# nubomedia/NUBOMEDIA-VCA

Measured on AMD Instinct MI355X. Metric: 1080p frames/sec/node (NuboFaceDetector); achieved HBM GB/s vs peak, higher is better.
Workload: dtype i32 rect sums / f32 products / f64 stage sums (u8 pixels)

## Files before the change

### nubomedia-vca_amd/csrc/device_records.h

```cpp
#pragma once
#include <stdint.h>
#include <stddef.h>

#if defined(__HIPCC__)
#define NVCA_HD __host__ __device__
#else
#define NVCA_HD
#endif

namespace nvca {

struct StageRec {
    int first, count; float thr;
    int flags;
    int thr_i;
    int vote_exp;
    int spec_run;
    int pad1;
};

struct ScaleRec {
    int    winw, winh;
    int    plane_off;
    int    pitch;
    int    endX, endY;
    int    eq[4];
    int    xpos_off, ypos_off;
    int    sq32;
    int    task_off;
    int    wpr;
    int    adaptive;
    double inv_area;
    double factor;
    const struct TStumpRec *trecs;
    const struct GNodeRec *grecs;
    const struct LStumpRec *lrecs;
};

struct GNodeRec {
    short dx[3][4], dy[3][4];
    float w[3];
    float thr;
    int left, right;
    int flags;
    int pad;
};
static_assert(sizeof(GNodeRec) == 80, "GNodeRec layout");

struct StripRec { int scale, iy0, nrows, ix0, ncols, pad0, pad1, pad2; };
struct TileRec {
    int scale, ix0, iy0, nx, ny;
    int x0, y0;
    int ncol, nrow;
    int span_x, span_y;
    int col_off, row_off;
    int pad_t;
    int pad0, pad1;
};
struct TStumpRec {
    int x0[3], x1[3], y0[3], y1[3];
    float w[3];
    int nrect;
    double thr, a0, a1;
    int a0i, a1i;
};
static_assert(sizeof(TStumpRec) == 96, "TStumpRec layout is read dword by dword in kernels_cascade_tile.hip");
struct alignas(16) LStumpRec {
    unsigned xx0, yy0, xx1, yy1, xx2, yy2;
    float w0, w1, w2, thr, a0, a1;
};
static_assert(sizeof(LStumpRec) == 48, "LStumpRec is read as three int4 in kernels_cascade_tile.hip");
struct DeepRec { int col_off, ncol, row_off, nrow, span_x, span_y, pad0, pad1; };
static constexpr int kDeepMaxSide = 64;
static constexpr int kDeepMaxSpan = 1280;
struct BandRec { int scale, iy0, ny, first_tile, ntiles, pad0, pad1, pad2; };
static constexpr int kTileWin = 32;
static constexpr int kTileRows = 16;
static constexpr int kTileSlots = kTileWin * kTileRows;
static constexpr int kTileThreads = kTileSlots;
static constexpr int kTilesPerCu = 3;
static constexpr int kTileWavesPerSimd = (kTilesPerCu * kTileThreads / 64 + 3) / 4;
static constexpr int kTileLdsBudget = 52 * 1024;
static_assert(kTilesPerCu * kTileLdsBudget <= 160 * 1024 && kTilesPerCu * kTileThreads <= 32 * 64, "tile residency per CU");
static constexpr int kTileMaxCols = 256;
NVCA_HD inline int tile_pitch(int ncol) { return ncol | 1; }
NVCA_HD inline int tile_lds_fixed()
{
    return kTileSlots * 8 + 2 * kTileSlots * 2 + 4 * kTileWin + 128 + kTileSlots * 8;
}
NVCA_HD inline int tile_lds_bytes(int ncol, int nrow, int span_x, int span_y)
{
    return 4 * nrow * tile_pitch(ncol) + 2 * ((span_x + 3) & ~3) + 2 * ((span_y + 3) & ~3) + tile_lds_fixed();
}

static constexpr int kStripMaxWin = 512;
static constexpr int kIntegralBand = 16;

struct PreGeom {
    int sw, sh, sstride, cn;
    int w, h, gpitch;
    int spitch;
    int nbands;
    size_t src_slot, gray_slot, sum_slot, band_slot;
};
struct YuvPlanes {
    int fmt, cstride, vstride, pad;
    long long off_y, off_u, off_v;
};
struct ResizeView {
    int mode, xmax;
    const int *xofs; const short *ialpha; const int *yofs; const short *ibeta;
};
struct PyrLevelDev {
    int szw, szh, gpitch, plane_off;
    long long gray_off;
    ResizeView tab;
};

struct TrkSlot {
    const uint8_t *src;
    uint8_t *prev;
    float *mhi;
    float ts, delbound;
    float seg;
    int threshold;
    int has_prev;
    int sstride;
    int min_area;
    long long max_area;
    YuvPlanes yuv;
};
struct CompAcc { int minx, miny, maxx, maxy, seed, pad; };
inline size_t tracker_count_offset(int w, int h, int batch) { return ((size_t)((w + 255) / 256) * h * batch + 63) & ~(size_t)63; }
inline size_t tracker_flag_bytes(int w, int h, int batch) { return tracker_count_offset(w, h, batch) + sizeof(int) * (size_t)batch; }

struct CascadeArgs {
    const int *sum; const unsigned long long *sqsum;
    size_t sum_slot;
    int spitch;
    const ScaleRec *scales; const StageRec *stages;
    const StripRec *strips; const int *pos;
    const int *order; int blocks_per_frame;
    const TileRec *tiles; const int *tile_order; int tile_blocks_per_frame;
    const unsigned short *tcoords; int tile_lds;
    const BandRec *bands; const int *band_order; int band_blocks_per_frame; int batch; int band_map;
    const DeepRec *deeprecs;
    int nscales;
    const unsigned *tasks; int ntasks;
    unsigned long long *failbits;
    double *vnf;
    int nstages; int pair_policy;
    int stage_order;
    int *stage_hint;
    int spec_pairs;
    int pair_max;
    const float *stage_thr;
    const int *stage_first;
    int deep_stage;
    int deep_lds;
    unsigned long long *deep;
    unsigned deep_cap;
    int key_sy, key_ss;
    unsigned long long *hits;
    unsigned hit_cap;
    const int *tilted;
    const float *galpha;
    const int *gcls_first;
    int stump_based;
#ifdef NVCA_STAMPS
    unsigned long long *dbg;
#endif
};

struct LbpWeakDev { int off[16]; int subset[8]; float leaf[2]; int pad[6]; };
static_assert(sizeof(LbpWeakDev) == 128, "LbpWeakDev is fetched with wide scalar loads");
struct LbpStageDev { int first, count; float thr; int pad; };
struct LbpLevelDev { int plane_off, szw, szh, nx, ny, step, wpr, bit_off, row_first, pad0, pad1, pad2; };
struct LbpTile { int level, tx, ty, pad; };
static constexpr int kLbpTileW = 32, kLbpTileH = 16;
NVCA_HD inline int lbp_tile_pitch(int ow) { return (kLbpTileW - 1) * 2 + ow + 1; }
NVCA_HD inline int lbp_tile_rows(int oh, int step) { return (kLbpTileH - 1) * step + oh + 1; }
struct LbpArgs {
    const int *sum;
    int P, TP;
    int ow, oh;
    const LbpLevelDev *levels; int nlev;
    const LbpStageDev *stages; int nstages;
    const LbpWeakDev *gweak, *tweak;
    const LbpTile *tiles; int ntiles;
    unsigned *bits, *bits2;
    int tile_stages;
    int nrows;
    int key_sy, key_ss;
    unsigned *cnt;
    unsigned *list[2]; unsigned list_cap;
    unsigned long long *hits; unsigned hit_cap;
};

struct RoiStep {
    const TStumpRec *trecs;
    int ex, ey, ew, eh;
    int startX, endX, startY, endY;
    int step, adaptive, job, key_step;
    int key_x0, key_dx, key_y0, key_dy;
    int szw, szh;
    int mode, xmax, xofs_off, yofs_off, ialpha_off, ibeta_off;
    double inv_area, ystep;
    int rej_off, rej_wpr;
};
struct RoiJobDev {
    const uint8_t *img; int w, h, stride;
    int first_step, nsteps, scale_image;
    const StageRec *stages; int nstages, pair_policy;
    int slot, pad;
};
static constexpr int kRoiMaxWin = 2048;

}
```

### nubomedia-vca_amd/csrc/kernels_cascade_tile.hip

```cpp
#include "launch.h"
#include "cascade_device.h"
#include <mutex>

namespace nvca {

template <class T> __device__ __forceinline__ T load_const(const T *p)
{
    static_assert(sizeof(T) % 4 == 0, "dword records only");
    typedef const __attribute__((address_space(4))) int CInt;
    CInt *q = (CInt *)p;
    T r;
    int *d = (int *)&r;
#pragma unroll
    for (int i = 0; i < (int)(sizeof(T) / 4); i++) d[i] = q[i];
    return r;
}

struct ScaleHot {
    int plane_off, pitch, eq[4], xpos_off, ypos_off, sq32, task_off, wpr, adaptive;
    double inv_area;
    const TStumpRec *trecs; const LStumpRec *lrecs;
};
__device__ __forceinline__ ScaleHot load_scale(const ScaleRec *p)
{
    typedef const __attribute__((address_space(4))) ScaleRec CScaleRec;
    CScaleRec *q = (CScaleRec *)p;
    ScaleHot h;
    h.plane_off = q->plane_off; h.pitch = q->pitch;
#pragma unroll
    for (int i = 0; i < 4; i++) h.eq[i] = q->eq[i];
    h.xpos_off = q->xpos_off; h.ypos_off = q->ypos_off; h.sq32 = q->sq32; h.task_off = q->task_off; h.wpr = q->wpr; h.adaptive = q->adaptive;
    h.inv_area = q->inv_area;
    h.trecs = q->trecs; h.lrecs = q->lrecs;
    return h;
}
struct TileScale {
    int pitch, xpos_off, ypos_off, wpr;
    const char *sum;
    double *vnf;
    const TStumpRec *trecs; const LStumpRec *lrecs;
};
__device__ __forceinline__ TileScale tile_scale(const CascadeArgs &a, const ScaleHot &h, int slot)
{
    TileScale ts;
    ts.pitch = h.pitch; ts.xpos_off = h.xpos_off; ts.ypos_off = h.ypos_off; ts.wpr = h.wpr;
    ts.sum = (const char *)(a.sum + (size_t)slot * a.sum_slot + h.plane_off);
    ts.vnf = a.vnf + ((size_t)slot * a.ntasks + h.task_off) * 64;
    ts.trecs = h.trecs; ts.lrecs = h.lrecs;
    return ts;
}


typedef int int16v __attribute__((ext_vector_type(16)));
typedef int int8v __attribute__((ext_vector_type(8)));
struct SRec { int16v a; int8v b; };
__device__ __forceinline__ SRec load_srec(const TStumpRec *p)
{
    SRec r;
    asm volatile("s_load_dwordx16 %0, %2, 0x0\n\ts_load_dwordx8 %1, %2, 0x40\n\ts_waitcnt lgkmcnt(0)"
                 : "=&s"(r.a), "=&s"(r.b) : "s"(p) : "memory");
    return r;
}
typedef __attribute__((address_space(1))) const void *gptr_t;
typedef __attribute__((address_space(3))) void *lptr_t;
typedef __attribute__((address_space(3))) const unsigned short lds_cu16;
typedef __attribute__((address_space(3))) const int lds_ci32;
#pragma clang diagnostic push
#pragma clang diagnostic ignored "-Wint-to-pointer-cast"
__device__ __forceinline__ unsigned lds_addr(const void *p) { return (unsigned)(unsigned long long)(lptr_t)p; }
__device__ __forceinline__ int lds_u16(unsigned a) { return *(lds_cu16 *)a; }
__device__ __forceinline__ int lds_sample(int r, int c)
{
    unsigned a;
    asm("v_lshl_add_u32 %0, %1, 2, %2" : "=v"(a) : "v"(r), "v"(c));
    return *(lds_ci32 *)a;
}
#pragma clang diagnostic pop
template <bool PAIR, class Sum>
__device__ __forceinline__ Sum tile_vote_s(unsigned cm, unsigned rm, double vnf, const SRec &f)
{
    const int share = f.a[15] >> 8;
    const int ca = lds_u16(cm + 2 * f.a[0]), cb = lds_u16(cm + 2 * f.a[3]);
    const int ra = lds_u16(rm + 2 * f.a[6]), rb = lds_u16(rm + 2 * f.a[9]);
    auto rs = [&](int x0, int x1, int y0, int y1, int sh) {
        int c0 = ca, c1 = cb, r0 = ra, r1 = rb;
        if (!(sh & 2)) { c0 = lds_u16(cm + 2 * x0); c1 = lds_u16(cm + 2 * x1); }
        if (!(sh & 1)) { r0 = lds_u16(rm + 2 * y0); r1 = lds_u16(rm + 2 * y1); }
        return lds_sample(r0, c0) - lds_sample(r0, c1) - lds_sample(r1, c0) + lds_sample(r1, c1);
    };
    const int s0 = lds_sample(ra, ca) - lds_sample(ra, cb) - lds_sample(rb, ca) + lds_sample(rb, cb);
    const int s1 = rs(f.a[1], f.a[4], f.a[7], f.a[10], share);
    const double t = __hiloint2double(f.b[1], f.b[0]) * vnf;
    const float w0 = __int_as_float(f.a[12]), w1 = __int_as_float(f.a[13]);
    double v;
    if (PAIR) {
        const float fs = (float)s0 * w0 + (float)s1 * w1;
        v = (double)fs;
    } else {
        v = (double)((float)s0 * w0);
        v += (double)((float)s1 * w1);
        if ((f.a[15] & 255) == 3) {
            const int s2 = rs(f.a[2], f.a[5], f.a[8], f.a[11], share >> 2);
            v += (double)((float)s2 * __int_as_float(f.a[14]));
        }
    }
    if (sizeof(Sum) == sizeof(int)) return (Sum)(v >= t ? f.b[7] : f.b[6]);
    const double a0 = __hiloint2double(f.b[3], f.b[2]), a1 = __hiloint2double(f.b[5], f.b[4]);
    return (Sum)(v >= t ? a1 : a0);
}
template <bool PAIR, class Sum = double>
__device__ __forceinline__ Sum tile_stage_sum(unsigned cm, unsigned rm, double vnf, const TStumpRec *recs, int j0, int count, int step)
{
    const TStumpRec *base = recs;
    asm("" : "+v"(cm), "+v"(rm));
    Sum sum = 0;
    for (int j = j0; j < count; j += step) sum += tile_vote_s<PAIR, Sum>(cm, rm, vnf, load_srec(base + j));
    return sum;
}
__device__ __forceinline__ bool tile_stage_pass(unsigned cm, unsigned rm, double vnf, const TStumpRec *recs, const StageRec &st, bool pair)
{
    if (st.flags & 4) {
        const int sum = pair ? tile_stage_sum<true, int>(cm, rm, vnf, recs + st.first, 0, st.count, 1) : tile_stage_sum<false, int>(cm, rm, vnf, recs + st.first, 0, st.count, 1);
        return sum >= st.thr_i;
    }
    const double sum = pair ? tile_stage_sum<true>(cm, rm, vnf, recs + st.first, 0, st.count, 1) : tile_stage_sum<false>(cm, rm, vnf, recs + st.first, 0, st.count, 1);
    return !(sum < (double)st.thr);
}

struct LRec { int4 a, b, c; };
__device__ __forceinline__ LRec load_lrec(const LStumpRec *p)
{
    const int4 *q = (const int4 *)p;
    LRec r; r.a = q[0]; r.b = q[1]; r.c = q[2];
    return r;
}
__device__ __forceinline__ int lane_rect(unsigned cm, unsigned rm, unsigned xx, unsigned yy)
{
    const int c0 = lds_u16(cm + (xx & 0xffffu)), c1 = lds_u16(cm + (xx >> 16));
    const int r0 = lds_u16(rm + (yy & 0xffffu)), r1 = lds_u16(rm + (yy >> 16));
    return lds_sample(r0, c0) - lds_sample(r0, c1) - lds_sample(r1, c0) + lds_sample(r1, c1);
}
__device__ __forceinline__ double lane_vote(unsigned cm, unsigned rm, double vnf, const LRec &f, int pair_policy)
{
    const int s0 = lane_rect(cm, rm, (unsigned)f.a.x, (unsigned)f.a.y);
    const int s1 = lane_rect(cm, rm, (unsigned)f.a.z, (unsigned)f.a.w);
    const double t = (double)__int_as_float(f.c.y) * vnf;
    const float p0 = (float)s0 * __int_as_float(f.b.z), p1 = (float)s1 * __int_as_float(f.b.w);
    double v = (double)p0;
    v += (double)p1;
    if (f.b.x) v += (double)((float)lane_rect(cm, rm, (unsigned)f.b.x, (unsigned)f.b.y) * __int_as_float(f.c.x));
    else if (pair_policy && f.b.y == 1) v = (double)(p0 + p1);
    return (double)__int_as_float(v >= t ? f.c.w : f.c.z);
}

#ifdef NVCA_STAMPS
#define NVCA_STAMP(a, tile, id) do { if (threadIdx.x == 0 && blockIdx.x < 64 && (tile) < 16 && (id) < 64 && (a).dbg) { unsigned long long t__; \
    asm volatile("s_memtime %0\n\ts_waitcnt lgkmcnt(0)" : "=s"(t__) :: "memory"); (a).dbg[((size_t)blockIdx.x * 16 + (tile)) * 64 + (id)] = t__; } } while (0)
#define NVCA_STAMP_VAL(a, tile, id, v) do { if (threadIdx.x == 0 && blockIdx.x < 64 && (tile) < 16 && (id) < 64 && (a).dbg) (a).dbg[((size_t)blockIdx.x * 16 + (tile)) * 64 + (id)] = (unsigned long long)(v); } while (0)
#else
#define NVCA_STAMP(a, tile, id) do { } while (0)
#define NVCA_STAMP_VAL(a, tile, id, v) do { } while (0)
#endif

struct TileLds {
    double *acc;
    unsigned short *q0, *winx, *winy; int *qn; double *vnf_s;
    unsigned short *cmap, *rmap; int *T; int pitchT;
    int tword;
    unsigned cmA, rmA;
};
__device__ __forceinline__ TileLds carve_tile(unsigned char *lds, const TileRec &t)
{
    TileLds L;
    L.acc = (double *)lds;
    L.q0 = (unsigned short *)(lds + kTileSlots * 8);
    L.winx = L.q0 + 2 * kTileSlots; L.winy = L.winx + kTileWin;
    L.qn = (int *)(L.winy + kTileWin);
    L.vnf_s = (double *)((unsigned char *)L.qn + 128);
    L.cmap = (unsigned short *)(L.vnf_s + kTileSlots);
    L.rmap = L.cmap + ((t.span_x + 3) & ~3);
    L.T = (int *)(L.rmap + ((t.span_y + 3) & ~3));
    L.pitchT = tile_pitch(t.ncol);
    L.tword = (int)(lds_addr(L.T) >> 2);
    L.cmA = lds_addr(L.cmap); L.rmA = lds_addr(L.rmap);
    return L;
}

struct TileCoords { int mapc, mapr, wx, wy; unsigned rowy, xc[4]; };
__device__ __forceinline__ TileCoords tile_coords(const CascadeArgs &a, const TileRec &t, const TileScale &sc)
{
    const int tid = threadIdx.x, lane = tid & 63, wave = tid >> 6;
    constexpr int NW = kTileThreads / 64;
    const unsigned short *__restrict__ cl = a.tcoords + t.col_off, *__restrict__ rl = a.tcoords + t.row_off;
    TileCoords c;
    c.mapc = tid < t.ncol ? (int)cl[tid] : -1;
    c.mapr = tid < t.nrow ? (int)rl[tid] : -1;
    c.wx = tid < t.nx ? a.pos[sc.xpos_off + t.ix0 + tid] : 0;
    c.wy = (tid >= 64 && tid < 64 + t.ny) ? a.pos[sc.ypos_off + t.iy0 + tid - 64] : 0;
    const int nmine = t.nrow > wave ? (t.nrow - wave + NW - 1) / NW : 0;
    c.rowy = 0u;
    if (lane < nmine) c.rowy = rl[wave + NW * lane];
#pragma unroll
    for (int k = 0; k < 4; k++) { const int q = lane + 64 * k; c.xc[k] = cl[q < t.ncol ? q : t.ncol - 1]; }
    return c;
}
__device__ __forceinline__ void tile_commit(const TileRec &t, const TileScale &sc, const TileLds &L, const TileCoords &c)
{
    const int tid = threadIdx.x, lane = tid & 63, wave = __builtin_amdgcn_readfirstlane(tid >> 6);
    constexpr int NW = kTileThreads / 64;
    const char *__restrict__ src = sc.sum;
    const int nmine = t.nrow > wave ? (t.nrow - wave + NW - 1) / NW : 0;
    const int nk = (t.ncol + 63) >> 6;
    for (int j = 0; j < nmine; j++) {
        const unsigned rb = (unsigned)__builtin_amdgcn_readlane((int)c.rowy, j) * (unsigned)sc.pitch * 4u;
        const char *rowp = src + rb;
        int *dst = L.T + (wave + NW * j) * L.pitchT;
#pragma unroll
        for (int k = 0; k < 4; k++)
            if (k < nk && lane + 64 * k < t.ncol)
                __builtin_amdgcn_global_load_lds((gptr_t)(rowp + 4u * c.xc[k]), (lptr_t)(dst + 64 * k), 4, 0, 0);
    }
    if (tid < 3) L.qn[tid] = 0;
    if (tid < t.nx) L.winx[tid] = (unsigned short)(c.wx - t.x0);
    if (tid >= 64 && tid < 64 + t.ny) L.winy[tid - 64] = (unsigned short)(c.wy - t.y0);
    if (c.mapc >= 0) L.cmap[c.mapc - t.x0] = (unsigned short)(tid * 4);
    if (c.mapr >= 0) L.rmap[c.mapr - t.y0] = (unsigned short)(L.tword + tid * L.pitchT);
}

__device__ __forceinline__ void queue_push_wave0(bool keep, int w, unsigned short *q, int *count)
{
    if (threadIdx.x >= 64) return;
    const int lane = threadIdx.x;
    const unsigned long long km = __ballot(keep);
    if (keep) q[__popcll(km & ((1ull << lane) - 1ull))] = (unsigned short)w;
    if (lane == 0) *count = __popcll(km);
}
__device__ __forceinline__ void queue_push(bool keep, int w, unsigned short *q, int *count)
{
    const int lane = threadIdx.x & 63;
    const unsigned long long km = __ballot(keep);
    if (km) {
        int wbase = 0;
        if (lane == 0) wbase = atomicAdd(count, __popcll(km));
        wbase = __shfl(wbase, 0);
        if (keep) q[wbase + __popcll(km & ((1ull << lane) - 1ull))] = (unsigned short)w;
    }
}

static constexpr int kStatStages = 6;
static constexpr int kPairMax = 32;
static_assert(7 * kPairMax <= kTileSlots && 64 + kTileRows <= kTileThreads && kTileRows <= kTileWin,
              "a round's seven accumulator rows fit the tile's accumulators; threads 64 .. 64 + kTileRows - 1 fill winy[kTileWin]");
template <bool VNF_LDS>
__device__ __forceinline__ void tile_stages(const CascadeArgs &a, const TileRec &t, const TileScale &sc, int slot, const TileLds &L, int ti = 0, int par = 0)
{
    const int tid = threadIdx.x, lane = tid & 63;
    const int wave = __builtin_amdgcn_readfirstlane(tid >> 6);
    const int *stat_r = L.qn + 4 + par * kStatStages;
    int *stat_w = L.qn + 4 + (par ^ 1) * kStatStages;
    constexpr int NW = kTileThreads / 64;
    const TStumpRec *urecs = sc.trecs;
    const double *__restrict__ vnfp = sc.vnf + (size_t)t.iy0 * sc.wpr * 64;
    auto vnf_of = [&](int w) {
        if (VNF_LDS) return L.vnf_s[w];
        const int ix = t.ix0 + (w & 31);
        return vnfp[((size_t)(w >> 5) * sc.wpr + (ix >> 6)) * 64 + (ix & 63)];
    };
    int *acci = (int *)L.acc;
    int cur = 0;
    int cin = 0;
    const int last = a.deep_stage < a.nstages ? a.deep_stage : a.nstages;
    const int m = (last < kStatStages ? last : kStatStages) - 1;
    const bool adapt = a.stage_order && m >= 2;
    unsigned ordpack = 0x54321u;
    if (adapt) {
        const unsigned o = (unsigned)__builtin_amdgcn_readfirstlane(stat_r[0]);
        unsigned seen = 0;
        for (int q = 0; q < m; q++) seen |= 1u << ((o >> (4 * q)) & 15u);
        if (seen == (2u << m) - 2u) ordpack = o;
    }
    int kpos = 0, prev = 0; unsigned entered = 0;
    auto stage_at = [&](int kp) { return __builtin_amdgcn_readfirstlane((adapt && kp < m) ? (int)((ordpack >> (4 * kp)) & 15u) : kp + 1); };
    struct I8 { int v[8]; };
    struct F8 { float v[8]; };
    const int s_first = last > 1 ? stage_at(0) : 0;
    StageRec st = load_const(a.stages + s_first);
    I8 F = load_const((const I8 *)(a.stage_first + s_first));
    F8 TH = load_const((const F8 *)(a.stage_thr + s_first));
    while (kpos < last - 1) {
        const bool in_prefix = adapt && kpos < m;
        const int s = stage_at(kpos);
        __syncthreads();
        NVCA_STAMP(a, ti, 8 + 8 * s);
        const int n = __builtin_amdgcn_readfirstlane(L.qn[cin]);
        if (adapt && tid == 0 && prev) stat_w[prev] |= n;
        if (n == 0) break;
        NVCA_STAMP_VAL(a, ti, 8 + 8 * s + 7, n);
        const int cout = cin == 2 ? 0 : cin + 1;
        if (tid == 0) L.qn[cout == 2 ? 0 : cout + 1] = 0;
        const unsigned short *qi = L.q0 + cur * kTileSlots;
        unsigned short *qo = L.q0 + (cur ^ 1) * kTileSlots;
        const bool pair = a.pair_policy && (st.flags & 1);
        int adv = 1;
        if (n <= a.pair_max && (st.flags & 2)) {
            const int G = 64 / n;
            int mm = 1;
            if (!in_prefix) {
                int lim = st.spec_run < last - s ? st.spec_run : last - s;
                if (lim > 7) lim = 7;
#pragma unroll
                for (int q = 1; q < 7; q++)
                    if (mm == q && q < lim && n * (F.v[q + 1] - F.v[0]) <= a.spec_pairs) mm = q + 1;
            }
            const int g0 = F.v[0];
            int g1 = F.v[1];
#pragma unroll
            for (int q = 2; q < 8; q++) if (mm >= q) g1 = F.v[q];
            const unsigned inv = 65535u / (unsigned)n + 1u;
            const int cc = (int)(((unsigned)lane * inv) >> 16), j = lane - cc * n;
            if (cc < G) {
                const int w = qi[j];
                const unsigned cm = L.cmA + 2 * L.winx[w & 31], rm = L.rmA + 2 * L.winy[w >> 5];
                const double vnf = vnf_of(w);
                for (int g = g0 + wave * G + cc; g < g1; g += NW * G) {
                    const LRec f = load_lrec(sc.lrecs + g);
                    const int r = (g >= F.v[1]) + (g >= F.v[2]) + (g >= F.v[3]) + (g >= F.v[4]) + (g >= F.v[5]) + (g >= F.v[6]);
                    atomicAdd(&L.acc[r * kPairMax + j], lane_vote(cm, rm, vnf, f, a.pair_policy));
                }
            }
            NVCA_STAMP(a, ti, 8 + 8 * s + 1);
            __syncthreads();
            NVCA_STAMP(a, ti, 8 + 8 * s + 2);
            bool pass = false; int w = 0;
            if (tid < n) {
                pass = true;
#pragma unroll
                for (int r = 0; r < 7; r++)
                    if (r < mm) {
                        const double sum = L.acc[r * kPairMax + tid];
                        L.acc[r * kPairMax + tid] = 0.;
                        pass = pass && !(sum < (double)TH.v[r]);
                    }
                w = qi[tid];
            }
            if (s < kStatStages && tid == 0) stat_w[s] = adapt ? n << 16 : n;
            queue_push_wave0(pass, w, qo, &L.qn[cout]);
            adv = mm;
            NVCA_STAMP(a, ti, 8 + 8 * s + 3);
        } else if (st.flags & 6) {
            const bool ints = (st.flags & 4) != 0;
            const int C = st.count;
            const int rem = n & 63, nfull = n >> 6;
            const bool rem_pair = rem > 0 && rem <= a.pair_max;
            const int Gr = rem_pair ? 64 / rem : 1;
            const int lead = (rem_pair ? nfull : (n + 63) >> 6) * C;
            const int items = lead + (rem_pair ? (C + Gr - 1) / Gr : 0), K = (items + NW - 1) / NW;
            const double vscale = ints ? __hiloint2double((1023 - st.vote_exp) << 20, 0) : 1.;
            int e = wave * K;
            const int e1 = e + K < items ? e + K : items;
            while (e < e1 && e < lead) {
                const int top = e1 < lead ? e1 : lead;
                const int wg = e / C, c0 = e - wg * C, c1 = (C - c0 < top - e) ? C : c0 + (top - e);
                const int i = wg * 64 + lane;
                if (i < n) {
                    const int w = qi[i];
                    const int xw = L.winx[w & 31], yw = L.winy[w >> 5];
                    const double vnf = vnf_of(w);
                    const unsigned cm = L.cmA + 2 * xw, rm = L.rmA + 2 * yw;
                    if (ints) {
                        const int v = pair ? tile_stage_sum<true, int>(cm, rm, vnf, urecs + st.first, c0, c1, 1) : tile_stage_sum<false, int>(cm, rm, vnf, urecs + st.first, c0, c1, 1);
                        atomicAdd(&acci[i], v);
                    } else {
                        const double v = pair ? tile_stage_sum<true, double>(cm, rm, vnf, urecs + st.first, c0, c1, 1) : tile_stage_sum<false, double>(cm, rm, vnf, urecs + st.first, c0, c1, 1);
                        atomicAdd(&L.acc[i], v);
                    }
                }
                e += c1 - c0;
            }
            if (e < e1) {
                const unsigned inv = 65535u / (unsigned)rem + 1u;
                const int cc = (int)(((unsigned)lane * inv) >> 16), j = lane - cc * rem;
                if (cc < Gr) {
                    const int i = nfull * 64 + j;
                    const int w = qi[i];
                    const unsigned cm = L.cmA + 2 * L.winx[w & 31], rm = L.rmA + 2 * L.winy[w >> 5];
                    const double vnf = vnf_of(w);
                    double sum = 0.;
                    for (int c = (e - lead) * Gr + cc; c < (e1 - lead) * Gr && c < C; c += Gr)
                        sum += lane_vote(cm, rm, vnf, load_lrec(sc.lrecs + st.first + c), a.pair_policy);
                    if (ints) atomicAdd(&acci[i], (int)(sum * vscale)); else atomicAdd(&L.acc[i], sum);
                }
            }
            NVCA_STAMP(a, ti, 8 + 8 * s + 1);
            __syncthreads();
            NVCA_STAMP(a, ti, 8 + 8 * s + 2);
            bool pass = false; int w = 0;
            if (tid < n) {
                if (ints) { const int sa = acci[tid]; acci[tid] = 0; pass = sa >= st.thr_i; }
                else { const double sa = L.acc[tid]; L.acc[tid] = 0.; pass = !(sa < (double)st.thr); }
                w = qi[tid];
            }
            if (s < kStatStages && tid == 0) stat_w[s] = adapt ? n << 16 : n;
            if (n <= 64) queue_push_wave0(pass, w, qo, &L.qn[cout]); else queue_push(pass, w, qo, &L.qn[cout]);
            NVCA_STAMP(a, ti, 8 + 8 * s + 3);
        } else {
            for (int base = 0; base < n; base += kTileThreads) {
                const int i = base + tid;
                bool pass = false; int w = 0;
                if (i < n) {
                    w = qi[i];
                    const int xw = L.winx[w & 31], yw = L.winy[w >> 5];
                    const double vnf = vnf_of(w);
                    pass = tile_stage_pass(L.cmA + 2 * xw, L.rmA + 2 * yw, vnf, urecs, st, pair);
                }
                queue_push(pass, w, qo, &L.qn[cout]);
            }
            if (tid == 0 && s < kStatStages) stat_w[s] = adapt ? n << 16 : n;
        }
        cur ^= 1; cin = cout;
        if (in_prefix) { prev = s; entered |= 1u << s; } else prev = 0;
        kpos += adv;
        if (kpos < last - 1) {
            const int sn = stage_at(kpos);
            st = load_const(a.stages + sn); F = load_const((const I8 *)(a.stage_first + sn)); TH = load_const((const F8 *)(a.stage_thr + sn));
        }
    }
    __syncthreads();
    NVCA_STAMP(a, ti, 6);
    const int nh = L.qn[cin];
    if (adapt && tid == 0) {
        if (prev) stat_w[prev] |= nh;
        int key[kStatStages - 1], id[kStatStages - 1];
        bool known = true;
#pragma unroll
        for (int q = 1; q < kStatStages; q++) {
            int v = stat_w[q];
            const int old = stat_r[q];
            if (q <= m && (!((entered >> q) & 1u) || ((v >> 16) < 16 && old != 0))) { v = old; stat_w[q] = v; }
            const int ent = v >> 16, pas = v & 0xffff, cnt = L.qn[4 + 2 * kStatStages - 1 + q] ;
            if (q <= m && ent == 0) known = false;
            const int killed = ent - pas > 0 ? ent - pas : 0;
            key[q - 1] = q > m ? 0x7fffffff : (killed ? (cnt * ent * 64) / killed : 0x7ffffff0);
            id[q - 1] = q;
        }
#pragma unroll
        for (int pass_i = 0; pass_i < kStatStages - 2; pass_i++)
#pragma unroll
            for (int q = 0; q + 1 < kStatStages - 1 - pass_i; q++)
                if (key[q] / 2 > key[q + 1]) { const int tk = key[q];        key[q] = key[q + 1]; key[q + 1] = tk; const int ti2 = id[q]; id[q] = id[q + 1]; id[q + 1] = ti2; }
        unsigned pack = 0;
#pragma unroll
        for (int q = 0; q < kStatStages - 1; q++) pack |= (unsigned)id[q] << (4 * q);
        stat_w[0] = known ? (int)pack : 0;
        if (known && a.stage_hint) {
#pragma unroll
            for (int q = 1; q < kStatStages; q++) a.stage_hint[q] = stat_w[q];
            a.stage_hint[0] = (int)pack;
        }
    }
    if (nh == 0) return;
    unsigned long long *list = last == a.nstages ? a.hits : a.deep;
    const unsigned cap = last == a.nstages ? a.hit_cap : a.deep_cap;
    if (tid == 0) L.qn[3] = (int)(unsigned)atomicAdd(list, (unsigned long long)nh);
    __syncthreads();
    const unsigned gb = (unsigned)L.qn[3];
    const unsigned short *qi = L.q0 + cur * kTileSlots;
    for (int i = tid; i < nh; i += kTileThreads) {
        const int w = qi[i], ix = t.ix0 + (w & 31);
        const unsigned key = ((unsigned)t.scale << a.key_ss) | ((unsigned)(t.iy0 + (w >> 5)) << a.key_sy) | (unsigned)ix;
        if (gb + i < cap) list[1 + gb + i] = ((unsigned long long)slot << 32) | key;
        if (VNF_LDS && last != a.nstages) sc.vnf[((size_t)(t.iy0 + (w >> 5)) * sc.wpr + (ix >> 6)) * 64 + (ix & 63)] = L.vnf_s[w];
    }
    NVCA_STAMP(a, ti, 7);
}

__device__ __forceinline__ void tile_prologue(const CascadeArgs &a, const TileLds &L)
{
    const int tid = threadIdx.x;
    L.acc[tid] = 0.;
    if (tid < 2 * kStatStages) L.qn[4 + tid] = (tid < kStatStages && a.stage_hint) ? a.stage_hint[tid] : 0;
    if (tid >= 1 && tid < kStatStages) L.qn[4 + 2 * kStatStages - 1 + tid] = tid < a.nstages ? a.stages[tid].count : 0;
}

__global__ __launch_bounds__(kTileThreads, kTileWavesPerSimd) void k_tile(CascadeArgs a)
{
    extern __shared__ __align__(16) unsigned char lds[];
    const int tid = threadIdx.x;
    const int slot = blockIdx.x / a.tile_blocks_per_frame;
    const int tidx = a.tile_order[blockIdx.x - slot * a.tile_blocks_per_frame];
    if (tidx < 0) return;
    const TileRec t = a.tiles[tidx];
    const ScaleHot sh = load_scale(a.scales + t.scale);
    const TileScale sc = tile_scale(a, sh, slot);
    const TileLds L = carve_tile(lds, t);
    const TileCoords tc = tile_coords(a, t, sc);
    tile_commit(t, sc, L, tc);
    tile_prologue(a, L);
    const unsigned long long *__restrict__ bits = a.failbits + (size_t)slot * a.ntasks + sh.task_off + (size_t)t.iy0 * sc.wpr;
    const int w = tid, ry = w >> 5, rx = w & 31;
    bool keep = false;
    if (ry < t.ny && rx < t.nx) {
        const int ix = t.ix0 + rx;
        const unsigned long long *rb = bits + (size_t)ry * sc.wpr;
        if (!((rb[ix >> 6] >> (ix & 63)) & 1ull)) keep = sh.adaptive ? visited(rb, ix) : true;
    }
    asm volatile("s_waitcnt vmcnt(0)" ::: "memory");
    __syncthreads();
    queue_push(keep, w, L.q0, &L.qn[0]);
    tile_stages<false>(a, t, sc, slot, L);
}

__global__ __launch_bounds__(kTileThreads, kTileWavesPerSimd) void k_band(CascadeArgs a)
{
    extern __shared__ __align__(16) unsigned char lds[];
    const int tid = threadIdx.x, lane = tid & 63;
    int bi = blockIdx.x / a.batch, slot = blockIdx.x - bi * a.batch;
    if (a.band_map) {
        const int xcd = blockIdx.x & 7, k = blockIdx.x >> 3;
        const int g = a.band_map;
        const int fi = k / (a.band_blocks_per_frame * g), r = k - fi * a.band_blocks_per_frame * g;
        bi = r / g; slot = xcd + 8 * (fi * g + (r - bi * g));
    }
    const BandRec b = load_const(a.bands + a.band_order[bi]);
    const ScaleHot sh = load_scale(a.scales + b.scale);
    const TileScale sc = tile_scale(a, sh, slot);
    const unsigned *__restrict__ sql = (const unsigned *)a.sqsum + (size_t)slot * 2 * a.sum_slot + sh.plane_off;
    const uint8_t *__restrict__ sqh = (const uint8_t *)((const unsigned *)a.sqsum + (size_t)slot * 2 * a.sum_slot + a.sum_slot) + sh.plane_off;
    const bool sq_lo_only = sh.sq32 != 0;
    const int ex0 = sh.eq[0] % sh.pitch, ey0 = sh.eq[0] / sh.pitch, ex1 = sh.eq[3] % sh.pitch, ey1 = sh.eq[3] / sh.pitch;
    const double inv_area = sh.inv_area;
    const bool adaptive_x = sh.adaptive != 0;
    const StageRec st0 = load_const(a.stages);
    const bool pair0 = a.pair_policy && (st0.flags & 1);
    static_assert(kTileSlots == kTileThreads, "one window per thread and tile");
    const int w = tid, ry = w >> 5, rx = w & 31;
    unsigned carry = 0;
    TileRec t = load_const(a.tiles + b.first_tile);
    TileCoords tc = tile_coords(a, t, sc);
    tile_prologue(a, carve_tile(lds, t));
    int oxw = 0, oyw = 0;
    if (ry < t.ny && rx < t.nx) { oxw = a.pos[sc.xpos_off + t.ix0 + rx]; oyw = a.pos[sc.ypos_off + t.iy0 + ry]; }
    for (int ti = 0; ti < b.ntiles; ti++) {
        __syncthreads();
        NVCA_STAMP(a, ti, 0);
        const TileLds L = carve_tile(lds, t);
        const bool active = ry < t.ny && rx < t.nx;
        int xw = oxw, yw = oyw;
        unsigned q0 = 0, q1 = 0, q2 = 0, q3 = 0, h0 = 0, h1 = 0, h2 = 0, h3 = 0;
        if (active) {
            xw -= t.x0; yw -= t.y0;
            const unsigned off = (unsigned)((t.y0 + yw) * sc.pitch + t.x0 + xw);
            const unsigned e0 = off + sh.eq[0], e1 = off + sh.eq[1], e2 = off + sh.eq[2], e3 = off + sh.eq[3];
            q0 = sql[e0]; q1 = sql[e1]; q2 = sql[e2]; q3 = sql[e3];
            if (!sq_lo_only) { h0 = sqh[e0]; h1 = sqh[e1]; h2 = sqh[e2]; h3 = sqh[e3]; }
        }
        NVCA_STAMP(a, ti, 1);
        tile_commit(t, sc, L, tc);
        if (tid < kStatStages) L.qn[4 + ((ti + 1) & 1) * kStatStages + tid] = 0;
        TileRec tn = t; TileCoords tcn = tc; int nxw = 0, nyw = 0;
        if (ti + 1 < b.ntiles) {
            tn = load_const(a.tiles + b.first_tile + ti + 1);
            tcn = tile_coords(a, tn, sc);
            if (ry < tn.ny && rx < tn.nx) { nxw = a.pos[sc.xpos_off + tn.ix0 + rx]; nyw = a.pos[sc.ypos_off + tn.iy0 + ry]; }
        }
        NVCA_STAMP(a, ti, 2);
        asm volatile("s_waitcnt vmcnt(0)" ::: "memory");
        __syncthreads();
        NVCA_STAMP(a, ti, 3);
        asm volatile("" : "+v"(h0), "+v"(h1), "+v"(h2), "+v"(h3));
        bool pass0 = false;
        if (active) {
            const int c0 = L.cmap[xw + ex0], c1 = L.cmap[xw + ex1], r0 = L.rmap[yw + ey0], r1 = L.rmap[yw + ey1];
            const int ws = lds_sample(r0, c0) - lds_sample(r0, c1) - lds_sample(r1, c0) + lds_sample(r1, c1);
            const double mean = (double)ws * inv_area;
            double vnf;
            if (sq_lo_only) vnf = (double)(unsigned)(q0 - q1 - q2 + q3);
            else vnf = (double)(((unsigned long long)h0 << 32) | q0) - (double)(((unsigned long long)h1 << 32) | q1) -
                       (double)(((unsigned long long)h2 << 32) | q2) + (double)(((unsigned long long)h3 << 32) | q3);
            vnf = vnf * inv_area - mean * mean;
            vnf = vnf >= 0. ? sqrt(vnf) : 1.;
            L.vnf_s[w] = vnf;
            pass0 = tile_stage_pass(L.cmA + 2 * xw, L.rmA + 2 * yw, vnf, sc.trecs, st0, pair0);
        }
        const unsigned long long fb = __ballot(active && !pass0);
        const unsigned R = lane < 32 ? (unsigned)fb : (unsigned)(fb >> 32);
        bool keep = false;
        if (active && !((R >> rx) & 1u)) {
            if (!adaptive_x) keep = true;
            else {
                int ones = 0;
                if (rx > 0) {
                    const unsigned mk = ~(R << (32 - rx));
                    ones = mk ? __clz((int)mk) : 32;
                    if (ones > rx) ones = rx;
                }
                const int cbit = (int)((carry >> (lane >> 5)) & 1u);
                const int parity = ones == rx ? ((rx + cbit) & 1) : (ones & 1);
                keep = !parity;
            }
        }
        {
            unsigned nc = 0;
#pragma unroll
            for (int h = 0; h < 2; h++) {
                const unsigned Rh = h ? (unsigned)(fb >> 32) : (unsigned)fb;
                const unsigned mk = ~(Rh << (32 - t.nx));
                int ones = mk ? __clz((int)mk) : 32;
                if (ones > t.nx) ones = t.nx;
                const unsigned p = ones == t.nx ? ((unsigned)t.nx + ((carry >> h) & 1u)) & 1u : (unsigned)ones & 1u;
                nc |= p << h;
            }
            carry = (unsigned)__builtin_amdgcn_readfirstlane((int)nc);
        }
        queue_push(keep, w, L.q0, &L.qn[0]);
        NVCA_STAMP(a, ti, 5);
        tile_stages<true>(a, t, sc, slot, L, ti, ti & 1);
        t = tn; tc = tcn; oxw = nxw; oyw = nyw;
    }
}

static int grant_lds(const void *fn, int which, int bytes, int *granted)
{
    if (bytes <= *granted) return 0;
    static std::mutex mu;
    static int dev_max[2][64] = {{0}};
    std::lock_guard<std::mutex> lk(mu);
    int dev = 0; (void)hipGetDevice(&dev); dev &= 63;
    if (bytes > dev_max[which][dev]) {
        const hipError_t e = hipFuncSetAttribute(fn, hipFuncAttributeMaxDynamicSharedMemorySize, bytes);
        if (e != hipSuccess) return (int)e;
        dev_max[which][dev] = bytes;
    }
    *granted = dev_max[which][dev];
    return 0;
}

int launch_tile(hipStream_t st, const CascadeArgs &a, int batch, int *lds_grant)
{
    if (batch <= 0 || a.ntasks <= 0 || a.tile_blocks_per_frame <= 0) return 0;
    if (int e = grant_lds(reinterpret_cast<const void *>(k_tile), 0, a.tile_lds, &lds_grant[0])) return e;
    NVCA_LAUNCH(k_tile, dim3((unsigned)a.tile_blocks_per_frame * (unsigned)batch), dim3(kTileThreads), (size_t)a.tile_lds, st, a);
    return 0;
}

int launch_band(hipStream_t st, const CascadeArgs &a, int batch, int *lds_grant)
{
    if (batch <= 0 || a.ntasks <= 0 || a.band_blocks_per_frame <= 0) return 0;
    if (int e = grant_lds(reinterpret_cast<const void *>(k_band), 1, a.tile_lds, &lds_grant[1])) return e;
    NVCA_LAUNCH(k_band, dim3((unsigned)a.band_blocks_per_frame * (unsigned)batch), dim3(kTileThreads), (size_t)a.tile_lds, st, a);
    return 0;
}

}
```

Before: 21240.

## Shrink tile window queues to 320 slots with overflow second pass

```diff
diff --git a/nubomedia-vca_amd/csrc/device_records.h b/nubomedia-vca_amd/csrc/device_records.h
--- a/nubomedia-vca_amd/csrc/device_records.h
+++ b/nubomedia-vca_amd/csrc/device_records.h
@@ -77,6 +77,9 @@
 static constexpr int kTileWin = 32;
 static constexpr int kTileRows = 16;
 static constexpr int kTileSlots = kTileWin * kTileRows;
+static constexpr int kTileQueue = 320;
+static_assert(kTileQueue % 64 == 0 && kTileQueue % kTileWin == 0 && kTileQueue <= kTileSlots && 2 * kTileQueue >= kTileSlots,
+              "whole waves and whole window rows per group; the two queues together take one push of every window of a tile");
 static constexpr int kTileThreads = kTileSlots;
 static constexpr int kTilesPerCu = 3;
 static constexpr int kTileWavesPerSimd = (kTilesPerCu * kTileThreads / 64 + 3) / 4;
@@ -86,7 +89,7 @@
 NVCA_HD inline int tile_pitch(int ncol) { return ncol | 1; }
 NVCA_HD inline int tile_lds_fixed()
 {
-    return kTileSlots * 8 + 2 * kTileSlots * 2 + 4 * kTileWin + 128 + kTileSlots * 8;
+    return kTileQueue * 8 + 2 * kTileQueue * 2 + 4 * kTileWin + 128 + kTileSlots * 8;
 }
 NVCA_HD inline int tile_lds_bytes(int ncol, int nrow, int span_x, int span_y)
 {
diff --git a/nubomedia-vca_amd/csrc/kernels_cascade_tile.hip b/nubomedia-vca_amd/csrc/kernels_cascade_tile.hip
--- a/nubomedia-vca_amd/csrc/kernels_cascade_tile.hip
+++ b/nubomedia-vca_amd/csrc/kernels_cascade_tile.hip
@@ -161,6 +161,12 @@
 #define NVCA_STAMP(a, tile, id) do { } while (0)
 #define NVCA_STAMP_VAL(a, tile, id, v) do { } while (0)
 #endif
+#ifdef NVCA_STAMPS
+#define NVCA_STAMP_QUEUED(a, n) do { if (threadIdx.x == 0 && (a).dbg) { atomicAdd(&(a).dbg[4], 1ull); if ((n) > 256) atomicAdd(&(a).dbg[64 + 4], 1ull); \
+    if ((n) > 320) atomicAdd(&(a).dbg[128 + 4], 1ull); if ((n) > 384) atomicAdd(&(a).dbg[192 + 4], 1ull); if ((n) > kTileQueue) atomicAdd(&(a).dbg[256 + 4], 1ull); } } while (0)
+#else
+#define NVCA_STAMP_QUEUED(a, n) do { } while (0)
+#endif
 
 struct TileLds {
     double *acc;
@@ -173,8 +179,8 @@
 {
     TileLds L;
     L.acc = (double *)lds;
-    L.q0 = (unsigned short *)(lds + kTileSlots * 8);
-    L.winx = L.q0 + 2 * kTileSlots; L.winy = L.winx + kTileWin;
+    L.q0 = (unsigned short *)(lds + kTileQueue * 8);
+    L.winx = L.q0 + 2 * kTileQueue; L.winy = L.winx + kTileWin;
     L.qn = (int *)(L.winy + kTileWin);
     L.vnf_s = (double *)((unsigned char *)L.qn + 128);
     L.cmap = (unsigned short *)(L.vnf_s + kTileSlots);
@@ -249,10 +255,12 @@
 
 static constexpr int kStatStages = 6;
 static constexpr int kPairMax = 32;
-static_assert(7 * kPairMax <= kTileSlots && 64 + kTileRows <= kTileThreads && kTileRows <= kTileWin,
+static constexpr int kKeepWord = 4 + 2 * kStatStages + kStatStages - 1;
+static_assert(kKeepWord + 2 * (kTileSlots - kTileQueue) / 64 <= 32, "the ballots fit the 32 counter words");
+static_assert(7 * kPairMax <= kTileQueue && 64 + kTileRows <= kTileThreads && kTileRows <= kTileWin,
               "a round's seven accumulator rows fit the tile's accumulators; threads 64 .. 64 + kTileRows - 1 fill winy[kTileWin]");
 template <bool VNF_LDS>
-__device__ __forceinline__ void tile_stages(const CascadeArgs &a, const TileRec &t, const TileScale &sc, int slot, const TileLds &L, int ti = 0, int par = 0)
+__device__ __forceinline__ bool tile_walk(const CascadeArgs &a, const TileRec &t, const TileScale &sc, int slot, const TileLds &L, bool keep, int grp, int ti, int par)
 {
     const int tid = threadIdx.x, lane = tid & 63;
     const int wave = __builtin_amdgcn_readfirstlane(tid >> 6);
@@ -267,8 +275,6 @@
         return vnfp[((size_t)(w >> 5) * sc.wpr + (ix >> 6)) * 64 + (ix & 63)];
     };
     int *acci = (int *)L.acc;
-    int cur = 0;
-    int cin = 0;
     const int last = a.deep_stage < a.nstages ? a.deep_stage : a.nstages;
     const int m = (last < kStatStages ? last : kStatStages) - 1;
     const bool adapt = a.stage_order && m >= 2;
@@ -279,10 +285,22 @@
         for (int q = 0; q < m; q++) seen |= 1u << ((o >> (4 * q)) & 15u);
         if (seen == (2u << m) - 2u) ordpack = o;
     }
-    int kpos = 0, prev = 0; unsigned entered = 0;
     auto stage_at = [&](int kp) { return __builtin_amdgcn_readfirstlane((adapt && kp < m) ? (int)((ordpack >> (4 * kp)) & 15u) : kp + 1); };
     struct I8 { int v[8]; };
     struct F8 { float v[8]; };
+    bool crowded = false;
+    const bool stats = grp == 0;
+    if (grp) {
+        __syncthreads();
+        if (tid < 3) L.qn[tid] = 0;
+        __syncthreads();
+        bool mine = false;
+        if (wave >= kTileQueue / 64) mine = (L.qn[kKeepWord + 2 * (wave - kTileQueue / 64) + (lane >> 5)] >> (lane & 31)) & 1;
+        queue_push(mine, tid, L.q0, &L.qn[0]);
+    }
+    int cur = 0;
+    int cin = 0;
+    int kpos = 0, prev = 0; unsigned entered = 0;
     const int s_first = last > 1 ? stage_at(0) : 0;
     StageRec st = load_const(a.stages + s_first);
     I8 F = load_const((const I8 *)(a.stage_first + s_first));
@@ -292,14 +310,27 @@
         const int s = stage_at(kpos);
         __syncthreads();
         NVCA_STAMP(a, ti, 8 + 8 * s);
-        const int n = __builtin_amdgcn_readfirstlane(L.qn[cin]);
-        if (adapt && tid == 0 && prev) stat_w[prev] |= n;
+        int n = __builtin_amdgcn_readfirstlane(L.qn[cin]);
+        if (kpos == 0 && stats) NVCA_STAMP_QUEUED(a, n);
+        if (n > kTileQueue) {
+            NVCA_STAMP_VAL(a, ti, 9, n);
+            crowded = true;
+            queue_push(keep && tid < kTileQueue, tid, L.q0, &L.qn[1]);
+            if (wave >= kTileQueue / 64) {
+                const unsigned long long km = __ballot(keep);
+                if (lane == 0) { L.qn[kKeepWord + 2 * (wave - kTileQueue / 64)] = (int)(unsigned)km; L.qn[kKeepWord + 2 * (wave - kTileQueue / 64) + 1] = (int)(unsigned)(km >> 32); }
+            }
+            cin = 1;
+            __syncthreads();
+            n = __builtin_amdgcn_readfirstlane(L.qn[1]);
+        }
+        if (adapt && stats && tid == 0 && prev) stat_w[prev] |= n;
         if (n == 0) break;
         NVCA_STAMP_VAL(a, ti, 8 + 8 * s + 7, n);
         const int cout = cin == 2 ? 0 : cin + 1;
         if (tid == 0) L.qn[cout == 2 ? 0 : cout + 1] = 0;
-        const unsigned short *qi = L.q0 + cur * kTileSlots;
-        unsigned short *qo = L.q0 + (cur ^ 1) * kTileSlots;
+        const unsigned short *qi = L.q0 + cur * kTileQueue;
+        unsigned short *qo = L.q0 + (cur ^ 1) * kTileQueue;
         const bool pair = a.pair_policy && (st.flags & 1);
         int adv = 1;
         if (n <= a.pair_max && (st.flags & 2)) {
@@ -343,7 +374,7 @@
                     }
                 w = qi[tid];
             }
-            if (s < kStatStages && tid == 0) stat_w[s] = adapt ? n << 16 : n;
+            if (s < kStatStages && stats && tid == 0) stat_w[s] = adapt ? n << 16 : n;
             queue_push_wave0(pass, w, qo, &L.qn[cout]);
             adv = mm;
             NVCA_STAMP(a, ti, 8 + 8 * s + 3);
@@ -400,7 +431,7 @@
                 else { const double sa = L.acc[tid]; L.acc[tid] = 0.; pass = !(sa < (double)st.thr); }
                 w = qi[tid];
             }
-            if (s < kStatStages && tid == 0) stat_w[s] = adapt ? n << 16 : n;
+            if (s < kStatStages && stats && tid == 0) stat_w[s] = adapt ? n << 16 : n;
             if (n <= 64) queue_push_wave0(pass, w, qo, &L.qn[cout]); else queue_push(pass, w, qo, &L.qn[cout]);
             NVCA_STAMP(a, ti, 8 + 8 * s + 3);
         } else {
@@ -415,7 +446,7 @@
                 }
                 queue_push(pass, w, qo, &L.qn[cout]);
             }
-            if (tid == 0 && s < kStatStages) stat_w[s] = adapt ? n << 16 : n;
+            if (tid == 0 && stats && s < kStatStages) stat_w[s] = adapt ? n << 16 : n;
         }
         cur ^= 1; cin = cout;
         if (in_prefix) { prev = s; entered |= 1u << s; } else prev = 0;
@@ -428,7 +459,7 @@
     __syncthreads();
     NVCA_STAMP(a, ti, 6);
     const int nh = L.qn[cin];
-    if (adapt && tid == 0) {
+    if (adapt && stats && tid == 0) {
         if (prev) stat_w[prev] |= nh;
         int key[kStatStages - 1], id[kStatStages - 1];
         bool known = true;
@@ -458,13 +489,13 @@
             a.stage_hint[0] = (int)pack;
         }
     }
-    if (nh == 0) return;
+    if (nh == 0) return crowded;
     unsigned long long *list = last == a.nstages ? a.hits : a.deep;
     const unsigned cap = last == a.nstages ? a.hit_cap : a.deep_cap;
     if (tid == 0) L.qn[3] = (int)(unsigned)atomicAdd(list, (unsigned long long)nh);
     __syncthreads();
     const unsigned gb = (unsigned)L.qn[3];
-    const unsigned short *qi = L.q0 + cur * kTileSlots;
+    const unsigned short *qi = L.q0 + cur * kTileQueue;
     for (int i = tid; i < nh; i += kTileThreads) {
         const int w = qi[i], ix = t.ix0 + (w & 31);
         const unsigned key = ((unsigned)t.scale << a.key_ss) | ((unsigned)(t.iy0 + (w >> 5)) << a.key_sy) | (unsigned)ix;
@@ -472,12 +503,19 @@
         if (VNF_LDS && last != a.nstages) sc.vnf[((size_t)(t.iy0 + (w >> 5)) * sc.wpr + (ix >> 6)) * 64 + (ix & 63)] = L.vnf_s[w];
     }
     NVCA_STAMP(a, ti, 7);
+    return crowded;
+}
+
+template <bool VNF_LDS>
+__device__ __forceinline__ void tile_stages(const CascadeArgs &a, const TileRec &t, const TileScale &sc, int slot, const TileLds &L, bool keep, int ti = 0, int par = 0)
+{
+    for (int grp = 0; tile_walk<VNF_LDS>(a, t, sc, slot, L, keep, grp, grp ? 16 : ti, par); grp++) { }
 }
 
 __device__ __forceinline__ void tile_prologue(const CascadeArgs &a, const TileLds &L)
 {
     const int tid = threadIdx.x;
-    L.acc[tid] = 0.;
+    if (tid < kTileQueue) L.acc[tid] = 0.;
     if (tid < 2 * kStatStages) L.qn[4 + tid] = (tid < kStatStages && a.stage_hint) ? a.stage_hint[tid] : 0;
     if (tid >= 1 && tid < kStatStages) L.qn[4 + 2 * kStatStages - 1 + tid] = tid < a.nstages ? a.stages[tid].count : 0;
 }
@@ -507,7 +545,7 @@
     asm volatile("s_waitcnt vmcnt(0)" ::: "memory");
     __syncthreads();
     queue_push(keep, w, L.q0, &L.qn[0]);
-    tile_stages<false>(a, t, sc, slot, L);
+    tile_stages<false>(a, t, sc, slot, L, keep);
 }
 
 __global__ __launch_bounds__(kTileThreads, kTileWavesPerSimd) void k_band(CascadeArgs a)
@@ -614,7 +652,7 @@
         }
         queue_push(keep, w, L.q0, &L.qn[0]);
         NVCA_STAMP(a, ti, 5);
-        tile_stages<true>(a, t, sc, slot, L, ti, ti & 1);
+        tile_stages<true>(a, t, sc, slot, L, keep, ti, ti & 1);
         t = tn; tc = tcn; oxw = nxw; oyw = nyw;
     }
 }
```

Result: no change. 21360, median of 6 (+0.6%).
